# jonassibbesen/rpvg

Hardware: AMD Instinct MI355X
Metric: read-pairs quantified/sec (higher is better)
Workload: dtype f64

## Files before the change

### rpvg_amd/csrc/bounded_search.hip

```cpp

#include "common.hpp"

#include <algorithm>
#include <cstdlib>
#include <map>
#include <memory>
#include <mutex>
#include <numeric>

using namespace rpvg_hip_detail;

namespace {
std::mutex g_search_gate_mutex;
const rpvg_hip_ctx * g_search_gate_owner = nullptr;
}

static bool searchLaunchesEarly() {
    static const bool early = RPVG_EXPERIMENT_ENV("RPVG_HIP_SEARCH_LAUNCH_EARLY") != nullptr;
    return early;
}

constexpr uint64_t kSearchGateRows = 1ull << 17;

static void searchGateEnter(rpvg_hip_ctx * ctx, hipStream_t stream, const uint64_t matrix_rows) {
    static const bool open_gate = RPVG_EXPERIMENT_ENV("RPVG_HIP_NO_SEARCH_GATE") != nullptr;
    ctx->search_gate_held = !open_gate && matrix_rows >= kSearchGateRows;
    if (!ctx->search_gate_held) return;
    hipEvent_t previous = nullptr;
    {
        std::lock_guard<std::mutex> lock(g_search_gate_mutex);
        if (g_search_gate_owner && g_search_gate_owner != ctx && g_search_gate_owner->device == ctx->device) {
            previous = g_search_gate_owner->search_done;
            (void) hipStreamWaitEvent(stream, previous, 0);
        }
    }
    if (previous && !searchLaunchesEarly()) (void) waitEvent(previous);
}

static void searchGateLeave(rpvg_hip_ctx * ctx, hipStream_t stream) {
    if (!ctx->search_gate_held) return;
    ctx->search_gate_held = false;
    std::lock_guard<std::mutex> lock(g_search_gate_mutex);
    (void) hipEventRecord(ctx->search_done, stream);
    g_search_gate_owner = ctx;
}

void searchGateForget(const rpvg_hip_ctx * ctx) {
    std::lock_guard<std::mutex> lock(g_search_gate_mutex);
    if (g_search_gate_owner == ctx) g_search_gate_owner = nullptr;
}

struct rpvg_hip_pair_posteriors {
    std::vector<uint64_t> pair_off;
    void * block = nullptr;
    bool block_pinned = false;
    const uint32_t * first = nullptr, * second = nullptr;
    const double * posterior = nullptr;
    ~rpvg_hip_pair_posteriors() {
        if (block && block_pinned) pinnedFree(block);
        else std::free(block);
    }
};

namespace {

constexpr uint32_t kLdsRows = 2048;
constexpr uint32_t kSmallRows = 512;
constexpr uint32_t kSmallRowLdsCols = 128;
constexpr uint32_t kRowLdsCols = 512;

__device__ __forceinline__ double waveSum(double v) { return waveSumF64(v); }

__device__ __forceinline__ double addLog(const double log_x, const double log_y) {
    return log_x > log_y ? log_x + log1p(exp(log_y - log_x)) : log_y + log1p(exp(log_x - log_y));
}


template <int kBlock, typename ValueFn>
__device__ __forceinline__ double blockLogSumExp(const uint32_t n, ValueFn value, double * scratch) {
    const double lowest = -1.7976931348623157e308;
    const int lane = threadIdx.x & 63, wave = threadIdx.x >> 6;
    double mx = lowest;
    for (uint32_t k = threadIdx.x; k < n; k += kBlock) mx = fmax(mx, value(k));
#pragma unroll
    for (int d = 32; d >= 1; d >>= 1) mx = fmax(mx, __shfl_xor(mx, d, 64));
    __syncthreads();
    if (lane == 0) scratch[wave] = mx;
    __syncthreads();
#pragma unroll
    for (int w2 = 0; w2 < kBlock / 64; ++w2) mx = fmax(mx, scratch[w2]);
    double sum = 0.0;
    for (uint32_t k = threadIdx.x; k < n; k += kBlock) {
        const double v = value(k);
        if (v > lowest) sum += exp(v - mx);
    }
    sum = waveSum(sum);
    __syncthreads();
    if (lane == 0) scratch[wave] = sum;
    __syncthreads();
    double total = 0.0;
#pragma unroll
    for (int w2 = 0; w2 < kBlock / 64; ++w2) total += scratch[w2];
    return (n == 0 || !(mx > lowest)) ? lowest : mx + log(total);
}

struct SearchArgs {
    const uint32_t * order;
    uint32_t count;
    const uint64_t * mat_val_off;
    const uint64_t * mat_row_off;
    const uint32_t * mat_fast;
    const uint32_t * mat_mid;
    const uint64_t * mat_rows;
    const uint32_t * mat_cols;
    const double * values;
    const double * rowmax;
    const double * row_count;
    const double * row_noise;
    const uint64_t * col_off;
// ... 1057 lines not shown
        pack.add(d_big_pair_part_off, big_pair_part_off.data(), M);
    }
    const uint32_t evals_word = (M + 1) & ~1u, tail_words = evals_word + 4;
    w.evals_word = evals_word;
    w.tail_words = tail_words;
    auto & d_tail = w.d_tail;
    pack.addZero(d_tail, tail_words);
    if (w.extra_u64_count) pack.add(w.d_extra_u64, w.extra_u64, w.extra_u64_count);
    if (w.extra_zero_bytes) pack.addZero(w.d_extra_zero, w.extra_zero_bytes);
    int span = ctx->spanBegin(FAM_H2D);
    ok(pack.commit(st));
    if (!column_counts) d_col_count.borrow(const_cast<uint32_t *>(groups->d_column_counts), col_off[M]);
    ctx->spanEnd(span);
    ctx->stats.h2d_bytes += static_cast<double>(M * 20 + col_off[M] * 4);
    ok(d_lf.alloc(col_off[M]));
    ok(d_marg.alloc(col_off[M]));
    ok(d_opt_raw.alloc(col_off[M]));
    ok(d_opt.alloc(col_off[M]));
    ok(d_col_order.alloc(col_off[M]));
    ok(d_out_first.alloc(pair_cap_off[M]));
    ok(d_out_second.alloc(pair_cap_off[M]));
    ok(d_out_value.alloc(pair_cap_off[M]));
    if (e != hipSuccess) {
        setError("rpvg_hip_bounded_pair_posteriors: %s", hipGetErrorString(e));
        return (e == hipErrorOutOfMemory) ? RPVG_HIP_ERR_ALLOC : RPVG_HIP_ERR_RUNTIME;
    }

    SearchArgs args;
    args.order = d_order.ptr;
    args.count = M;
    args.mat_val_off = groups->mat_val_off.ptr;
    args.mat_row_off = groups->mat_row_off.ptr;
    args.mat_fast = groups->mat_fast.ptr;
    args.mat_mid = groups->mat_mid.ptr;
    args.mat_rows = groups->mat_rows.ptr;
    args.mat_cols = groups->mat_cols.ptr;
    args.values = groups->values.ptr;
    args.rowmax = groups->rowmax.ptr;
    args.row_count = groups->row_count.ptr;
    args.row_noise = groups->row_noise.ptr;
    args.col_off = d_col_off.ptr;
    args.col_count = d_col_count.ptr;
    args.pair_cap_off = d_pair_cap_off.ptr;
    args.min_log_likelihood_diff = std::log(min_rel_likelihood);
    args.log_freq = d_lf.ptr;
    args.marginal = d_marg.ptr;
    args.optimistic_raw = d_opt_raw.ptr;
    args.optimistic = d_opt.ptr;
    args.col_order = d_col_order.ptr;
    args.out_first = d_out_first.ptr;
    args.out_second = d_out_second.ptr;
    args.out_value = d_out_value.ptr;
    args.out_count = d_tail.ptr;

    args.log_evals = reinterpret_cast<unsigned long long *>(d_tail.ptr + evals_word);
    auto & d_part_marg = w.d_part_marg; auto & d_part_opt = w.d_part_opt; auto & d_part_pair = w.d_part_pair; auto & d_seq = w.d_seq;
    if (num_big > 0) {
        ok(d_part_marg.alloc(col_part_total));
        ok(d_part_opt.alloc(col_part_total));
        ok(d_part_pair.alloc(pair_part_total));
        ok(d_seq.alloc(pair_cap_off[M]));
    }
    if (e != hipSuccess) {
        setError("rpvg_hip_bounded_pair_posteriors: %s", hipGetErrorString(e));
        return (e == hipErrorOutOfMemory) ? RPVG_HIP_ERR_ALLOC : RPVG_HIP_ERR_RUNTIME;
    }

    static const int search_streams = []() {
        const char * env = RPVG_EXPERIMENT_ENV("RPVG_HIP_SEARCH_STREAMS");
        return env ? std::max(1, std::min(3, std::atoi(env))) : 3;
    }();
    hipStream_t s_medium = search_streams == 1 ? st : ctx->aux[0];
    hipStream_t s_small = search_streams == 1 ? st : (search_streams == 2 ? ctx->aux[0] : ctx->aux[1]);
    const bool side_kernels = M > num_big;
    const bool runs_behind_search = static_cast<bool>(groups->held_back_runs) && pair_tiles && num_big == M;
    if (!runs_behind_search) {
        ok(groups->waitCollapse(st));
        if (groups->collapse_done && !searchLaunchesEarly()) {
            HostScope wait_scope("search: wait for the collapse of the matrices");
            ok(waitEvent(groups->collapse_done));
        }
    }
    span = ctx->spanBegin(FAM_LOGLIK);
    searchGateEnter(ctx, st, std::accumulate(groups->h_num_rows.begin(), groups->h_num_rows.end(), uint64_t(0)));
    if (side_kernels) ok(ctx->forkAux());
    if (num_big > 0) {
        TableWork tw;
        tw.item_matrix = d_item_matrix.ptr;
        tw.item_col = d_item_col.ptr;
        tw.item_chunk = d_item_chunk.ptr;
        tw.count = static_cast<uint32_t>(item_matrix.size());
        tw.mat_val_off = groups->mat_val_off.ptr;
        tw.mat_row_off = groups->mat_row_off.ptr;
        tw.mat_fast = groups->mat_fast.ptr;
        tw.mat_mid = groups->mat_mid.ptr;
        tw.mat_rows = groups->mat_rows.ptr;
        tw.mat_cols = groups->mat_cols.ptr;
        tw.values = groups->values.ptr;
        tw.rowmax = groups->rowmax.ptr;
        tw.row_count = groups->row_count.ptr;
        tw.row_noise = groups->row_noise.ptr;
        tw.big_col_part_off = d_big_col_part_off.ptr;
        tw.big_pair_part_off = d_big_pair_part_off.ptr;
        tw.part_marginal = d_part_marg.ptr;
        tw.part_optimistic = d_part_opt.ptr;
        tw.part_pair = d_part_pair.ptr;
        tw.log_evals = args.log_evals;
        if (pair_tiles) {
            PairTileWork pw;
            pw.item_matrix = d_item_matrix.ptr;
            pw.item_chunk = d_item_chunk.ptr;
            pw.item_tiles = d_item_col.ptr;
            pw.chunk_rows = chunk_rows;
            pw.count = tw.count;
            pw.mat_val_off = groups->mat_val_off.ptr;
            pw.mat_row_off = groups->mat_row_off.ptr;
            pw.mat_fast = groups->mat_fast.ptr;
            pw.mat_mid = groups->mat_mid.ptr;
            pw.mat_rows = groups->mat_rows.ptr;
            pw.mat_cols = groups->mat_cols.ptr;
            pw.values = groups->values.ptr;
            pw.row_count = groups->row_count.ptr;
            pw.row_noise = groups->row_noise.ptr;
            pw.col_part_off = d_big_col_part_off.ptr;
            pw.pair_part_off = d_big_pair_part_off.ptr;
            pw.part_marginal = d_part_marg.ptr;
            pw.part_pair = d_part_pair.ptr;
            pw.log_evals = args.log_evals;
#ifdef RPVG_HIP_EXPERIMENTS
            pw.debug_skip = RPVG_EXPERIMENT_ENV("RPVG_HIP_PAIR_DEBUG") ? static_cast<uint32_t>(std::atoi(RPVG_EXPERIMENT_ENV("RPVG_HIP_PAIR_DEBUG"))) : 0u;
#endif
            static const size_t tile_lds_bytes = []() {
                const char * env = RPVG_EXPERIMENT_ENV("RPVG_HIP_PAIR_LDS_KB");
                return std::max<size_t>(kTileLdsDoubles * sizeof(double), env ? static_cast<size_t>(std::atoi(env)) * 1024 : 0);
            }();
            if (tile_lds_bytes > 64 * 1024) {
                RPVG_HIP_CHECK(hipFuncSetAttribute(reinterpret_cast<const void *>(&pairTile2Kernel), hipFuncAttributeMaxDynamicSharedMemorySize, static_cast<int>(tile_lds_bytes)));
            }
            const int tile_span = ctx->spanBegin(FAM_TILE, st);
            pairTile2Kernel<<<dim3(pw.count), dim3(kTileBlock), tile_lds_bytes, st>>>(pw);
            ctx->spanEnd(tile_span);
#ifdef RPVG_HIP_EXPERIMENTS
            for (int k = RPVG_EXPERIMENT_ENV("RPVG_HIP_PAIR_REPEAT") ? std::atoi(RPVG_EXPERIMENT_ENV("RPVG_HIP_PAIR_REPEAT")) : 0; k > 0; --k) {
                pairTile2Kernel<<<dim3(pw.count), dim3(kTileBlock), tile_lds_bytes, st>>>(pw);
            }
#endif
        } else {
            pairTableKernel<<<dim3(((tw.count + 7) / 8) * 8), dim3(256), 0, st>>>(tw);
        }
        if (runs_behind_search && e == hipSuccess) {
            if (groups->collapse_done) {
                HostScope wait_scope("search: wait for the runs of the matrices' collapse");
                ok(searchLaunchesEarly() ? hipStreamWaitEvent(st, groups->collapse_done, 0) : waitEvent(groups->collapse_done));
            }
            rpvg_hip_groups::SearchSums sums;
            sums.part_pair = d_part_pair.ptr;
            sums.part_marginal = d_part_marg.ptr;
            sums.pair_part_off = d_big_pair_part_off.ptr;
            sums.col_part_off = d_big_col_part_off.ptr;
            sums.chunk_rows = chunk_rows;
            ok(groups->held_back_runs(st, &sums));
            groups->held_back_runs = nullptr;
        }

        ResolveArgs ra;
        ra.big_matrix = d_order.ptr;
        ra.count = num_big;
        ra.mat_rows = groups->mat_rows.ptr;
        ra.mat_cols = groups->mat_cols.ptr;
        ra.chunk_rows = chunk_rows;
        ra.col_off = d_col_off.ptr;
        ra.col_count = d_col_count.ptr;
        ra.pair_cap_off = d_pair_cap_off.ptr;
        ra.big_col_part_off = d_big_col_part_off.ptr;
        ra.big_pair_part_off = d_big_pair_part_off.ptr;
        ra.part_marginal = d_part_marg.ptr;
        ra.part_optimistic = d_part_opt.ptr;
        ra.part_pair = d_part_pair.ptr;
        ra.min_log_likelihood_diff = args.min_log_likelihood_diff;
        ra.log_freq = d_lf.ptr;
        ra.marginal = d_marg.ptr;
        ra.col_order = d_col_order.ptr;
        ra.seq_value = d_seq.ptr;
        ra.out_first = d_out_first.ptr;
        ra.out_second = d_out_second.ptr;
        ra.out_value = d_out_value.ptr;
        ra.out_count = d_tail.ptr;
        resolveTableKernel<<<dim3(num_big), dim3(256), 0, st>>>(ra);
    }
    args.row_lds_cols = kRowLdsCols;
    auto search_lds_bytes = [](uint32_t stage_rows, uint32_t row_cols) { return static_cast<size_t>((kTileFirst + 1) * stage_rows + kTileFirst * row_cols) * sizeof(double); };
    {
        static std::once_flag once;
        std::call_once(once, [&]() {
            (void) hipFuncSetAttribute(reinterpret_cast<const void *>(&boundedSearchKernel<1024, 64>), hipFuncAttributeMaxDynamicSharedMemorySize,
                                       static_cast<int>(search_lds_bytes(kLdsRows, kRowLdsCols)));
        });
    }
    if (num_medium > 0) {
        args.order = d_order.ptr + num_big;
        args.count = num_medium;
        args.stage_rows = kLdsRows;
        boundedSearchKernel<1024, 64><<<dim3(num_medium), dim3(1024), search_lds_bytes(kLdsRows, kRowLdsCols), s_medium>>>(args);
    }
    if (M > num_big + num_medium) {
        args.order = d_order.ptr + num_big + num_medium;
        args.count = M - num_big - num_medium;
        args.stage_rows = kSmallRows;
        args.row_lds_cols = kSmallRowLdsCols;
        boundedSearchKernel<256, 16><<<dim3(args.count), dim3(256), search_lds_bytes(kSmallRows, kSmallRowLdsCols), s_small>>>(args);
    }
    if (side_kernels) ok(ctx->joinAux());
    ctx->spanEnd(span);
    ctx->stats.loglik_launches += (num_big > 0 ? 2 : 0) + (num_medium > 0) + (M > num_big + num_medium);
    ok(hipGetLastError());
    if (e != hipSuccess) {
        setError("rpvg_hip_bounded_pair_posteriors: %s", hipGetErrorString(e));
        (void) hipStreamSynchronize(st);
        return RPVG_HIP_ERR_RUNTIME;
    }
    return RPVG_HIP_OK;
}

void leavePairSearch(rpvg_hip_ctx * ctx) { searchGateLeave(ctx, ctx->stream); }

void accountPairSearch(rpvg_hip_ctx * ctx, const rpvg_hip_groups * groups, const PairSearchWork & w, const unsigned long long log_evals,
                       const uint64_t kept_pairs) {
    ctx->stats.loglik_evals += static_cast<double>(log_evals);
    for (uint32_t i = 0; i < w.M; ++i) {
        const double G = groups->h_num_cols[w.order[i]];
        ctx->stats.search_pairs_possible += G * (G + 1) / 2;
        if (i < w.num_big) ctx->stats.search_pairs_table += G * (G + 1) / 2;
    }
    ctx->stats.search_pairs_kept += static_cast<double>(kept_pairs);
}

}

extern "C" int rpvg_hip_bounded_pair_posteriors(rpvg_hip_ctx * ctx, const rpvg_hip_groups * groups,
                                                const uint32_t * column_counts, double min_rel_likelihood,
                                                rpvg_hip_pair_posteriors ** result_out) {
    RPVG_REQUIRE(ctx && groups && result_out, "rpvg_hip_bounded_pair_posteriors: NULL argument");
    *result_out = nullptr;
    RPVG_REQUIRE(min_rel_likelihood > 0, "rpvg_hip_bounded_pair_posteriors: min_rel_likelihood must be positive");
    const uint32_t M = groups->num_matrices;
    rpvg_hip_pair_posteriors * res = new (std::nothrow) rpvg_hip_pair_posteriors();
    if (!res) {
        setError("rpvg_hip_bounded_pair_posteriors: out of host memory");
        return RPVG_HIP_ERR_ALLOC;
    }
    res->pair_off.assign(M + 1, 0);
    if (M == 0) {
        *result_out = res;
        return RPVG_HIP_OK;
    }
    if (!column_counts && !groups->d_column_counts) {
        delete res;
        setError("rpvg_hip_bounded_pair_posteriors: column_counts is NULL");
        return RPVG_HIP_ERR_INVALID;
    }

    std::lock_guard<std::mutex> lock(ctx->mutex);
    PairSearchWork w;
    {
        const int rc = queuePairSearch(ctx, groups, column_counts, min_rel_likelihood, w);
        if (rc != RPVG_HIP_OK) {
            delete res;
            return rc;
        }
    }
    hipError_t e = hipSuccess;
    hipStream_t st = ctx->stream;
    auto ok = [&](hipError_t r) { if (e == hipSuccess) e = r; return e == hipSuccess; };
    std::unique_ptr<HostScope> scope;
    const std::vector<uint64_t> & pair_cap_off = w.pair_cap_off;
    const uint32_t evals_word = w.evals_word, tail_words = w.tail_words;
    auto & d_tail = w.d_tail; auto & d_pair_cap_off = w.d_pair_cap_off; auto & d_out_first = w.d_out_first;
    auto & d_out_second = w.d_out_second; auto & d_out_value = w.d_out_value;
    DeviceBuffer<uint64_t> d_pair_off;

    const char * with_counts_env = std::getenv("RPVG_HIP_PAIRS_WITH_COUNTS");
    const size_t kPairsWithTheCounts = with_counts_env ? static_cast<size_t>(std::atof(with_counts_env)) : (size_t(1) << 20);
    const size_t tail_bytes = tail_words * sizeof(uint32_t), tail_room = (tail_bytes + 255) & ~size_t(255);
    const size_t block_capacity = static_cast<size_t>(pair_cap_off[M]) * 16;
    const size_t first_copy = tail_room + std::min(block_capacity, kPairsWithTheCounts);
    DeviceBuffer<unsigned char> d_result;
    ok(d_pair_off.alloc(M + 1));
    ok(d_result.alloc(tail_room + block_capacity));
    void * host_result = nullptr;
    if (e == hipSuccess && pinnedAlloc(&host_result, first_copy) != hipSuccess) e = hipErrorOutOfMemory;
    if (e == hipSuccess) {
        const bool check_build = !groups->build_checked && groups->build_error_flag.ptr;
        pairOffsetsKernel<<<dim3(1), dim3(1024), 0, st>>>(M, d_tail.ptr, d_pair_off.ptr, check_build ? groups->build_error_flag.ptr : nullptr,
                                                         d_tail.ptr + evals_word + 2, reinterpret_cast<uint32_t *>(d_result.ptr), tail_words);
        compactPairsBlockKernel<<<dim3(M), dim3(64), 0, st>>>(M, d_pair_cap_off.ptr, d_pair_off.ptr, d_out_first.ptr, d_out_second.ptr,
                                                             d_out_value.ptr, d_result.ptr + tail_room);
        ok(hipGetLastError());
        ok(hipMemcpyAsync(host_result, d_result.ptr, first_copy, hipMemcpyDeviceToHost, st));
    }
    searchGateLeave(ctx, st);
    scope.reset(new HostScope("bounded search: wait for the kernels"));
    ok(waitStream(st));
    if (e == hipSuccess) {
        const uint32_t * counts = static_cast<const uint32_t *>(host_result);
        unsigned long long log_evals = 0;
        std::memcpy(&log_evals, counts + evals_word, sizeof(log_evals));
        const uint32_t build_bad = counts[evals_word + 2];
// ... 58 lines not shown
```

### rpvg_amd/csrc/common.hpp

```cpp
#ifndef RPVG_HIP_COMMON_HPP
#define RPVG_HIP_COMMON_HPP

#include <hip/hip_runtime.h>

#include <algorithm>
#include <chrono>
#include <cstdarg>
#include <cstdint>
#include <cstdio>
#include <cstdlib>
#include <cstring>
#include <memory>
#include <mutex>
#include <new>
#include <string>
#include <functional>
#include <vector>

#include "../../include/rpvg_hip.h"

namespace rpvg_hip_detail {

void setError(const char * fmt, ...);

// ... 415 lines not shown
    }
}

constexpr int kCollapseKeyFractionBits = 22;
constexpr int kCollapseProjectionBits = kCollapseKeyFractionBits + 2;
constexpr int kCollapseLargestBits = 20;
constexpr int kCollapseLargestFractionBits = 27;
constexpr int kCollapseMatrixShift = kCollapseProjectionBits + kCollapseLargestBits;
constexpr uint32_t kCollapseMaxMatrices = 1u << 20;

__host__ __device__ inline double collapseWeight(const uint32_t column) {
    return static_cast<double>(((column * 0x9E3779B1u) >> 8) & 0xFFFFu) * (1.0 / 32768.0);
}

__host__ __device__ inline uint64_t collapseSortKey(const uint32_t matrix, const double key, const double largest) {
    const double k = key < 0.0 ? 0.0 : (key > 3.999999 ? 3.999999 : key);
    const double l = largest < 0.0 ? 0.0 : (largest > 0.999999 ? 0.999999 : largest);
    return (static_cast<uint64_t>(matrix) << kCollapseMatrixShift) |
           (static_cast<uint64_t>(k * static_cast<double>(1ull << kCollapseKeyFractionBits)) << kCollapseLargestBits) |
           (static_cast<uint64_t>(l * static_cast<double>(1ull << kCollapseLargestFractionBits)) & ((1ull << kCollapseLargestBits) - 1));
}

__device__ __forceinline__ double mulRounded(const double a, const double b) {
#pragma clang fp contract(off)
    return a * b;
}
__device__ __forceinline__ double addRounded(const double a, const double b) {
#pragma clang fp contract(off)
    return a + b;
}

template <int BLOCK>
__device__ __forceinline__ uint32_t blockExclusiveSum(const uint32_t v, uint32_t & total, uint32_t * scratch) {
    const int lane = threadIdx.x & 63, wave = threadIdx.x >> 6;
    uint32_t incl = v;
#pragma unroll
    for (int d = 1; d < 64; d <<= 1) {
        const uint32_t up = __shfl_up(incl, d, 64);
        if (lane >= d) incl += up;
    }
    __syncthreads();
    if (lane == 63) scratch[wave] = incl;
    __syncthreads();
    uint32_t before = 0, all = 0;
#pragma unroll
    for (int w = 0; w < BLOCK / 64; ++w) {
        if (w < wave) before += scratch[w];
        all += scratch[w];
    }
    total = all;
    return before + incl - v;
}

enum KernelFamily { FAM_EM_SPARSE = 0, FAM_EM_DENSE, FAM_LOGLIK, FAM_BUILD, FAM_H2D, FAM_COLLAPSE, FAM_EM_KERNEL, FAM_GIBBS, FAM_TILE, FAM_COUNT };

struct TimedSpan {
    hipEvent_t start, stop;
    int family;
    int sub;
};

struct TimedInterval {
    double start_ms, stop_ms;
    int family;
    uint64_t clock;
};

}

namespace rpvg_hip_detail {
struct SubsetEmHints {
    double subsets_per_matrix = 0, list_per_path = 0, rows_per_row = 0, entries_per_entry = 0;
    bool retry = false;
    unsigned long long retry_subsets = 0, retry_list_length = 0, retry_rows = 0, retry_entries = 0;
};
}

struct rpvg_hip_ctx {
    static constexpr int kAuxStreams = 6;
    rpvg_hip_detail::SubsetEmHints subset_hints;
    bool search_gate_held = false;
    int device = 0;
    hipStream_t stream = nullptr;
    hipStream_t aux[kAuxStreams] = {};
    int aux_count = kAuxStreams;
    hipStream_t grid_stream[2] = {nullptr, nullptr};
    hipEvent_t grid_ready = nullptr;
    hipStream_t collapse_stream = nullptr;
    hipStream_t copy_stream = nullptr;
    hipEvent_t copied = nullptr;
    hipEvent_t fork_event = nullptr;
    hipEvent_t search_done = nullptr;
    hipEvent_t join_event[kAuxStreams] = {};
    hipError_t forkAux();
    hipError_t joinAux();
    hipError_t joinAuxOnHost();
    hipDeviceProp_t props;
    std::mutex mutex;
    void * comm = nullptr;
    int comm_world = 1, comm_rank = 0;
    int allReduceSumF64(double * device_buf, uint64_t n);
    std::vector<rpvg_hip_detail::TimedSpan> spans;
    std::vector<hipStream_t> span_streams;
    int span_level = 2;
    int open_spans = 0;
    void accountSpan(const rpvg_hip_detail::TimedSpan & span, const void * clock_base, uint64_t clock_id);
    void foldFinishedSpans();
    std::vector<rpvg_hip_detail::TimedInterval> intervals;
    rpvg_hip_kernel_stats stats;

    int spanBegin(int family, hipStream_t on = nullptr, int sub = -1);
    void spanEnd(int idx);
    int foldSpans();
};

namespace rpvg_hip_detail {
struct PathSourcesPending {
    DeviceBuffer<uint64_t> d_path_source_off;
    DeviceBuffer<uint32_t> d_source_id, d_sizes;
    DeviceBuffer<uint16_t> d_source_id16;
    DeviceBuffer<unsigned long long> d_arena;
    unsigned long long arena_words = 0, num_sources = 0, num_sources_narrow = 0;
    void * h_sizes = nullptr;
    uint32_t K = 0;
    bool copied = false, queued = false;
    ~PathSourcesPending() { if (h_sizes) pinnedFree(h_sizes); }
};
}

struct rpvg_hip_batch {
    uint32_t num_clusters = 0;
    uint64_t num_rows = 0, num_entries = 0, num_paths = 0;
    std::vector<uint64_t> h_cluster_row_off, h_cluster_path_off, h_cluster_ent_off;
    rpvg_hip_detail::DeviceBuffer<uint64_t> cluster_row_off;
    rpvg_hip_detail::DeviceBuffer<uint64_t> cluster_path_off;
    rpvg_hip_detail::DeviceBuffer<double> row_count;
    rpvg_hip_detail::DeviceBuffer<double> row_noise;
    rpvg_hip_detail::DeviceBuffer<uint64_t> row_ent_off;
    rpvg_hip_detail::DeviceBuffer<uint32_t> ent_path;
    rpvg_hip_detail::DeviceBuffer<double> ent_prob;
    std::vector<double> h_cluster_total;
    bool has_source_columns = false;
    rpvg_hip_detail::DeviceBuffer<uint32_t> path_group_id;
    rpvg_hip_detail::DeviceBuffer<uint64_t> cluster_src_off;
    rpvg_hip_detail::DeviceBuffer<uint32_t> src_col_count;
    rpvg_hip_detail::DeviceBuffer<uint32_t> src_col_end;
    rpvg_hip_detail::DeviceBuffer<uint32_t> src_col_path;
    std::vector<uint64_t> h_cluster_src_off;
    std::vector<uint32_t> h_src_num_cols, h_src_col_paths, h_src_max_col_paths;
    struct UploadInProgress {
        rpvg_hip_detail::DeviceBuffer<uint32_t> d_row_count_u32, d_row_grp_off32, d_grp_idx_off32;
        rpvg_hip_detail::DeviceBuffer<uint64_t> d_row_grp_off, d_grp_idx_off;
        rpvg_hip_detail::DeviceBuffer<double> d_grp_prob;
        rpvg_hip_detail::DeviceBuffer<uint8_t> d_row_grp_count8, d_grp_idx_count8;
        rpvg_hip_detail::DeviceBuffer<uint16_t> d_path_idx16, d_row_noise16;
        rpvg_hip_detail::DeviceBuffer<double> d_row_noise_table;
        rpvg_hip_detail::DeviceBuffer<uint8_t> d_row_count8;
        rpvg_hip_detail::DeviceBuffer<uint32_t> d_escape_row, d_escape_count;
        uint64_t num_groups = 0;
        rpvg_hip_detail::PathSourcesPending path_sources;
        rpvg_hip_detail::DeviceBuffer<unsigned long long> d_first_bad_row;
        rpvg_hip_detail::DeviceBuffer<double> d_cluster_total;
        rpvg_hip_detail::DeviceBuffer<uint64_t> d_cluster_ent_off;
        rpvg_hip_detail::DeviceBuffer<unsigned char> scan_scratch_rows, scan_scratch_groups;
        void * h_results = nullptr;
        hipEvent_t finished = nullptr;
// ... 126 lines not shown
    uint32_t num_fused = 0;
    hipEvent_t filled = nullptr, collapsed = nullptr, collapse_sorted = nullptr;
    ~EmSolveWork() {
        if (filled) (void) hipEventDestroy(filled);
        if (collapsed) (void) hipEventDestroy(collapsed);
        if (collapse_sorted) (void) hipEventDestroy(collapse_sorted);
    }
};
size_t emQueuesBytes();
uint32_t emFillSegmentRows();

struct EmGridControl {
    uint32_t done;
    uint32_t iterations;
    uint32_t conv_its;
    uint32_t viol;
    uint32_t error;
    uint32_t arrived;
};

struct EmGridProblem {
    uint32_t problem, columns;
    uint32_t rows, entries;
    uint32_t merged, pad;
    uint64_t row_base, ent_base, col_begin;
    double total_mass, zero_mass;
};

struct EmGridStorage {
    const uint32_t * prow_off;
    const double * prow_count;
    const double * merged_count;
    const double * prow_noise;
    const uint32_t * pent_col;
    const double * pent_val;
    double * abundances;
    double * noise_count;
    uint32_t * iterations;
    const EmFusedDense * fused = nullptr;
    uint32_t num_fused = 0;
};

uint64_t emGridMinWork();
bool emGridDenseRoute(uint32_t columns, uint32_t rows, uint32_t entries);
int runEmGridProblems(rpvg_hip_ctx * ctx, hipStream_t st, const EmGridProblem * problems, uint32_t count, const EmGridStorage & storage,
                      uint32_t max_em_its, double max_rel_em_conv);

struct DenseEmRun {
    const double * matrix = nullptr;
    uint64_t num_rows = 0;
    uint32_t num_cols = 0;
    uint64_t ld = 0;
    const double * counts = nullptr;
    double total_count = 0, zero_mass = 0;
    uint32_t max_em_its = 0;
    double max_rel_em_conv = 0;
    bool sharded = false;
    DeviceBuffer<double> d_a;
    EmGridControl control = {};
};
int emDenseIterate(rpvg_hip_ctx * ctx, const char * who, DenseEmRun & run);

int queueEmSolve(rpvg_hip_ctx * ctx, const rpvg_hip_batch * batch, const EmProblemList & list, uint32_t max_em_its,
                 double max_rel_em_conv, const EmOutputs & out, EmSolveWork & work, bool fill_only, double collapse_precision = 0.0);
void accountEmSolve(rpvg_hip_ctx * ctx, uint32_t P, const uint64_t * col_off, const uint32_t * kept_rows, const uint32_t * kept_entries,
                    const uint32_t * iterations);

struct PairSearchWork {
    uint32_t M = 0, num_big = 0, evals_word = 0, tail_words = 0;
    std::vector<uint32_t> order;
    std::vector<uint64_t> col_off, pair_cap_off;
    DeviceBuffer<uint32_t> d_order, d_col_count, d_col_order, d_out_first, d_out_second, d_item_matrix, d_item_col, d_item_chunk;
    DeviceBuffer<uint32_t> d_tail;
    DeviceBuffer<uint64_t> d_col_off, d_pair_cap_off, d_big_col_part_off, d_big_pair_part_off;
    DeviceBuffer<double> d_lf, d_marg, d_opt_raw, d_opt, d_out_value, d_part_marg, d_part_opt, d_part_pair, d_seq;
    UploadPack pack;
    const uint64_t * extra_u64 = nullptr;
    size_t extra_u64_count = 0, extra_zero_bytes = 0;
    DeviceBuffer<uint64_t> d_extra_u64;
    DeviceBuffer<unsigned char> d_extra_zero;
};
int queuePairSearch(rpvg_hip_ctx * ctx, const rpvg_hip_groups * groups, const uint32_t * column_counts, double min_rel_likelihood,
                    PairSearchWork & w);
void leavePairSearch(rpvg_hip_ctx * ctx);
void accountPairSearch(rpvg_hip_ctx * ctx, const rpvg_hip_groups * groups, const PairSearchWork & w, unsigned long long log_evals, uint64_t kept_pairs);

struct CsrCollapseInput {
    uint32_t num_problems_bound = 0;
    const uint32_t * num_problems_dev = nullptr;
    uint64_t rows_capacity = 0;
    const uint64_t * row_base = nullptr;
    const uint64_t * ent_base = nullptr;
    const uint32_t * kept_rows = nullptr;
    const uint64_t * col_off = nullptr;
    const uint32_t * prow_off = nullptr;
    const double * prow_count = nullptr;
    const double * prow_noise = nullptr;
    const uint32_t * pent_col = nullptr;
    const double * pent_val = nullptr;
    uint32_t num_items_bound = 0;
    const uint32_t * num_items_dev = nullptr;
    const uint64_t * seg_first = nullptr;
    const uint32_t * item_problem = nullptr;
    uint32_t segment_rows = 0;
    uint64_t max_rows_bound = 0;
};
struct CsrCollapseWork {
    DeviceBuffer<double> merged_count;
    DeviceBuffer<uint32_t> problem_merged;
    DeviceBuffer<uint32_t> info;
    std::shared_ptr<void> temporaries;
};
hipError_t queueCsrCollapse(rpvg_hip_ctx * ctx, const CsrCollapseInput & in, double precision, CsrCollapseWork & work, hipStream_t stream,
                            hipEvent_t sorted = nullptr);

hipError_t queueClusterTotals(hipStream_t stream, uint32_t num_clusters, const uint64_t * d_cluster_row_off, const uint32_t * d_row_count_u32, double * d_totals);
hipError_t queuePathSourceCopies(rpvg_hip_ctx * ctx, rpvg_hip_batch * b, const rpvg_cluster_batch * hb, PathSourcesPending & pending);
hipError_t queuePathSourceKernels(rpvg_hip_ctx * ctx, rpvg_hip_batch * b, PathSourcesPending & pending, hipStream_t stream);
hipError_t reservePathSources(rpvg_hip_batch * b, uint32_t num_clusters, uint64_t num_paths, uint64_t num_sources, PathSourcesPending & pending);
int finishPathSources(rpvg_hip_batch * b, PathSourcesPending & pending);

hipError_t queueRowCollapse(rpvg_hip_ctx * ctx, rpvg_hip_groups * groups, uint64_t total_rows, double precision, hipStream_t stream, bool hold_back_runs = false);
}

#endif
```

### rpvg_amd/csrc/context.hip

```cpp

#include "common.hpp"

#include <hipcub/hipcub.hpp>

#include <sys/prctl.h>
#include <time.h>

#include <algorithm>
#include <thread>

#include <map>

namespace rpvg_hip_detail {

static thread_local char g_last_error[1024] = "";

void setError(const char * fmt, ...) {
    va_list ap;
    va_start(ap, fmt);
    vsnprintf(g_last_error, sizeof(g_last_error), fmt, ap);
    va_end(ap);
}

namespace {
// ... 443 lines not shown
template <typename GrpOff>
__global__ void expandGroupsKernel(const uint64_t num_groups, const uint64_t num_entries, const GrpOff * __restrict__ grp_idx_off,
                                   const double * __restrict__ grp_prob, double * __restrict__ ent_prob) {
    const uint64_t g = blockIdx.x * static_cast<uint64_t>(blockDim.x) + threadIdx.x;
    if (g >= num_groups) return;
    const double p = grp_prob[g];
    for (uint64_t e = grp_idx_off[g]; e < min(static_cast<uint64_t>(grp_idx_off[g + 1]), num_entries); ++e) ent_prob[e] = p;
}

template <typename RowOff, typename GrpOff>
__global__ void rowMetaKernel(const uint64_t num_rows, const uint64_t num_groups, const RowOff * __restrict__ row_grp_off,
                              const GrpOff * __restrict__ grp_idx_off, const uint32_t * __restrict__ row_count_u32,
                              uint64_t * __restrict__ row_ent_off, double * __restrict__ row_count) {
    const uint64_t r = blockIdx.x * static_cast<uint64_t>(blockDim.x) + threadIdx.x;
    if (r > num_rows) return;
    row_ent_off[r] = grp_idx_off[min(static_cast<uint64_t>(row_grp_off[r]), num_groups)];
    if (r < num_rows) row_count[r] = static_cast<double>(row_count_u32[r]);
}

template <typename RowOff, typename GrpOff>
__global__ void validateRowsKernel(const uint64_t num_rows, const uint64_t num_groups, const uint64_t num_entries, const uint32_t num_clusters,
                                   const uint64_t * __restrict__ cluster_row_off, const uint64_t * __restrict__ cluster_path_off,
                                   const RowOff * __restrict__ row_grp_off, const GrpOff * __restrict__ grp_idx_off,
                                   const double * __restrict__ row_noise, const uint32_t * __restrict__ path_idx,
                                   unsigned long long * __restrict__ first_bad_row) {
    const uint64_t r = blockIdx.x * static_cast<uint64_t>(blockDim.x) + threadIdx.x;
    if (r >= num_rows) return;
    bool good = true;
    const uint64_t g0 = row_grp_off[r], g1 = row_grp_off[r + 1];
    good = g0 <= g1 && g1 <= num_groups;
    const double nz = row_noise[r];
    good = good && nz > 0 && nz <= 1;
    if (good) {
        uint32_t lo = 0, hi = num_clusters;
        while (hi - lo > 1) {
            const uint32_t mid = lo + (hi - lo) / 2;
            if (cluster_row_off[mid] <= r) lo = mid;
            else hi = mid;
        }
        const uint64_t n_paths = cluster_path_off[lo + 1] - cluster_path_off[lo];
        uint64_t e = grp_idx_off[g0];
        good = e <= num_entries;
        for (uint64_t g = g0; good && g < g1; ++g) {
            const uint64_t e1 = grp_idx_off[g + 1];
            good = e <= e1 && e1 <= num_entries;
            for (; good && e < e1; ++e) good = path_idx[e] < n_paths;
        }
    }
    if (!good) atomicMin(first_bad_row, static_cast<unsigned long long>(r));
}

extern "C" {

int rpvg_hip_device_count(int * count) {
    RPVG_REQUIRE(count != nullptr, "rpvg_hip_device_count: count is NULL");
    int n = 0;
    hipError_t e = hipGetDeviceCount(&n);
    if (e != hipSuccess) {
        setError("hipGetDeviceCount failed: %s", hipGetErrorString(e));
        *count = 0;
        return RPVG_HIP_ERR_NO_DEVICE;
    }
    *count = n;
    return RPVG_HIP_OK;
}

namespace {
hipError_t createMainStream(hipStream_t * stream, const bool highest_priority) {
    const char * env = RPVG_EXPERIMENT_ENV("RPVG_HIP_MAIN_PRIORITY");
    if (!highest_priority && (!env || std::atoi(env) == 0)) return hipStreamCreateWithFlags(stream, hipStreamNonBlocking);
    int least = 0, greatest = 0;
    if (hipDeviceGetStreamPriorityRange(&least, &greatest) != hipSuccess || least == greatest) {
        (void) hipGetLastError();
        return hipStreamCreateWithFlags(stream, hipStreamNonBlocking);
    }
    return hipStreamCreateWithPriority(stream, hipStreamNonBlocking, greatest);
}

bool ownQueueForMainStream(const bool uploader, const int side_streams) {
    static const bool pooled = std::getenv("RPVG_HIP_POOLED_MAIN_QUEUE") != nullptr && std::atoi(std::getenv("RPVG_HIP_POOLED_MAIN_QUEUE")) != 0;
    return !uploader && side_streams < rpvg_hip_ctx::kAuxStreams && !pooled;
}

hipError_t createOwnQueueStream(hipStream_t * stream, const int num_cus) {
    uint32_t every_cu[32];
    for (uint32_t & word : every_cu) word = 0xffffffffu;
    const uint32_t words = static_cast<uint32_t>(std::min(32, std::max(1, (num_cus + 31) / 32)));
    hipError_t e = hipExtStreamCreateWithCUMask(stream, words, every_cu);
    if (e != hipSuccess) {
        (void) hipGetLastError();
        e = hipStreamCreateWithFlags(stream, hipStreamNonBlocking);
    }
    return e;
}

int createContext(int device, bool uploader, int side_streams, rpvg_hip_ctx ** ctx_out);
}

int rpvg_hip_create(int device, rpvg_hip_ctx ** ctx_out) { return createContext(device, false, rpvg_hip_ctx::kAuxStreams, ctx_out); }

int rpvg_hip_create_uploader(int device, rpvg_hip_ctx ** ctx_out) { return createContext(device, true, 1, ctx_out); }

int rpvg_hip_create_with_streams(int device, int side_streams, rpvg_hip_ctx ** ctx_out) {
    RPVG_REQUIRE(side_streams >= 1 && side_streams <= rpvg_hip_ctx::kAuxStreams, "rpvg_hip_create_with_streams: 1 to %d side streams", rpvg_hip_ctx::kAuxStreams);
    return createContext(device, false, side_streams, ctx_out);
}

namespace {
int createContext(int device, const bool uploader, const int side_streams, rpvg_hip_ctx ** ctx_out) {
    RPVG_REQUIRE(ctx_out != nullptr, "rpvg_hip_create: ctx_out is NULL");
    *ctx_out = nullptr;
    int n = 0;
    hipError_t e = hipGetDeviceCount(&n);
    if (e != hipSuccess || n <= 0) {
        setError("rpvg_hip_create: no HIP device available (%s); this engine has no CPU fallback",
                 e != hipSuccess ? hipGetErrorString(e) : "device count is 0");
        return RPVG_HIP_ERR_NO_DEVICE;
    }
    RPVG_REQUIRE(device >= 0 && device < n, "rpvg_hip_create: device %d out of range [0, %d)", device, n);
    rpvg_hip_ctx * ctx = new (std::nothrow) rpvg_hip_ctx();
    if (!ctx) {
        setError("rpvg_hip_create: out of host memory");
        return RPVG_HIP_ERR_ALLOC;
    }
    ctx->device = device;
    memset(&ctx->stats, 0, sizeof(ctx->stats));
    {
        const char * env = std::getenv("RPVG_HIP_SPANS");
        ctx->span_level = env ? std::max(0, std::min(2, std::atoi(env))) : ((uploader || side_streams < rpvg_hip_ctx::kAuxStreams) ? 1 : 2);
    }
    if ((e = hipSetDevice(device)) != hipSuccess || (e = hipGetDeviceProperties(&ctx->props, device)) != hipSuccess ||
        (e = ownQueueForMainStream(uploader, side_streams) ? createOwnQueueStream(&ctx->stream, ctx->props.multiProcessorCount) : createMainStream(&ctx->stream, uploader)) != hipSuccess) {
        setError("rpvg_hip_create: %s", hipGetErrorString(e));
        delete ctx;
        return RPVG_HIP_ERR_RUNTIME;
    }
    ctx->aux_count = side_streams;
    for (int i = 0; i < rpvg_hip_ctx::kAuxStreams && e == hipSuccess; ++i) {
        if (i < side_streams) {
            e = hipStreamCreateWithFlags(&ctx->aux[i], hipStreamNonBlocking);
            if (e == hipSuccess) e = hipEventCreateWithFlags(&ctx->join_event[i], hipEventDisableTiming);
        } else {
            ctx->aux[i] = ctx->aux[i % side_streams];
        }
    }
    if (e == hipSuccess) e = createMainStream(&ctx->collapse_stream, RPVG_EXPERIMENT_ENV("RPVG_HIP_COLLAPSE_PRIORITY") == nullptr || std::atoi(RPVG_EXPERIMENT_ENV("RPVG_HIP_COLLAPSE_PRIORITY")) != 0);
    if (e == hipSuccess) e = hipEventCreateWithFlags(&ctx->fork_event, hipEventDisableTiming);
    if (e == hipSuccess) e = hipEventCreateWithFlags(&ctx->search_done, hipEventDisableTiming);
    if (e == hipSuccess) e = hipStreamCreateWithFlags(&ctx->copy_stream, hipStreamNonBlocking);
    if (e == hipSuccess) e = hipEventCreateWithFlags(&ctx->copied, hipEventDisableTiming);
    if (e == hipSuccess) {
        registerCopyStream(ctx->stream, ctx->copy_stream, ctx->copied);
        for (int i = 0; i < ctx->aux_count; ++i) registerCopyStream(ctx->aux[i], ctx->copy_stream, ctx->copied);
    }
    if (e != hipSuccess) {
        setError("rpvg_hip_create: %s", hipGetErrorString(e));
        delete ctx;
        return RPVG_HIP_ERR_RUNTIME;
    }
    if (strncmp(ctx->props.gcnArchName, "gfx950", 6) != 0) {
        setError("rpvg_hip_create: device %d is %s; this library is built for gfx950 only", device, ctx->props.gcnArchName);
        (void) hipStreamDestroy(ctx->stream);
        delete ctx;
        return RPVG_HIP_ERR_NO_DEVICE;
    }
    {
        std::lock_guard<std::mutex> lock(g_pool_mutex);
        g_device_contexts[device]++;
    }
    *ctx_out = ctx;
    return RPVG_HIP_OK;
}
}

void rpvg_hip_destroy(rpvg_hip_ctx * ctx) {
    if (!ctx) return;
    const bool trace = std::getenv("RPVG_AMD_TRACE_EXIT") != nullptr;
#define RPVG_EXIT_STEP(what) do { if (trace) std::fprintf(stderr, "[exit]   rpvg_hip_destroy: %s\n", what); } while (0)
    RPVG_EXIT_STEP("begin");
    (void) hipSetDevice(ctx->device);
    (void) ctx->foldSpans();
    RPVG_EXIT_STEP("spans folded");
    (void) rpvg_hip_comm_destroy(ctx);
    if (ctx->stream) forgetCopyStream(ctx->stream);
    for (int i = 0; i < ctx->aux_count; ++i) {
        if (ctx->aux[i]) forgetCopyStream(ctx->aux[i]);
    }
    if (ctx->copy_stream) {
        (void) hipStreamSynchronize(ctx->copy_stream);
        (void) hipStreamDestroy(ctx->copy_stream);
    }
    RPVG_EXIT_STEP("copy stream destroyed");
    if (ctx->copied) (void) hipEventDestroy(ctx->copied);
    if (ctx->stream) (void) hipStreamSynchronize(ctx->stream);
    for (int i = 0; i < ctx->aux_count; ++i) {
        if (ctx->aux[i]) (void) hipStreamSynchronize(ctx->aux[i]);
    }
    if (ctx->collapse_stream) (void) hipStreamSynchronize(ctx->collapse_stream);
    RPVG_EXIT_STEP("streams drained");
    for (int i = 0; i < ctx->aux_count; ++i) {
        if (ctx->aux[i]) (void) hipStreamDestroy(ctx->aux[i]);
        RPVG_EXIT_STEP("a side stream destroyed");
        if (ctx->join_event[i]) (void) hipEventDestroy(ctx->join_event[i]);
    }
    if (ctx->collapse_stream) (void) hipStreamDestroy(ctx->collapse_stream);
    RPVG_EXIT_STEP("side and collapse streams destroyed");
    if (ctx->stream) (void) hipStreamDestroy(ctx->stream);
    RPVG_EXIT_STEP("main stream destroyed");
    if (ctx->fork_event) (void) hipEventDestroy(ctx->fork_event);
    for (hipStream_t grid_stream : ctx->grid_stream) {
        if (grid_stream) {
            (void) hipStreamSynchronize(grid_stream);
            (void) hipStreamDestroy(grid_stream);
        }
    }
// ... 897 lines not shown
```

### rpvg_amd/csrc/subset_em.hip

```cpp

#include "common.hpp"

#include <cmath>
#include <memory>

using namespace rpvg_hip_detail;

namespace {

constexpr uint32_t kMaxSelected = 1024;

struct MergedList {
    const uint32_t * a;
    const uint32_t * b;
    uint32_t na, nb, i, j;
    __device__ __forceinline__ MergedList(const uint32_t * a_in, uint32_t na_in, const uint32_t * b_in, uint32_t nb_in)
        : a(a_in), b(b_in), na(na_in), nb(nb_in), i(0), j(0) {}
    __device__ __forceinline__ bool done() const { return i >= na && j >= nb; }
    __device__ __forceinline__ uint32_t next() {
        if (j >= nb || (i < na && a[i] <= b[j])) return a[i++];
        return b[j++];
    }
};

// ... 790 lines not shown
    ok(d_slot_columns.alloc(slots));
    ok(d_slot_weight.alloc(slots));
    ok(d_totals.alloc(sizeof(MatrixTotals) * M));
    ok(d_bases.alloc(sizeof(MatrixTotals) * M));
    DeviceBuffer<uint32_t> d_big_matrices;
    ok(d_big_matrices.alloc(M));
    DeviceBuffer<uint32_t> d_sub_cluster, d_path, d_col_path, d_iters, d_kept_rows, d_kept_entries;
    DeviceBuffer<double> d_sub_weight, d_abund, d_noise, d_total;
    DeviceBuffer<uint64_t> d_path_off, d_col_off, d_row_base, d_ent_base, d_subset_off, d_seg_first;
    DeviceBuffer<uint32_t> d_item_problem;
    ok(d_sub_cluster.alloc(cap_subsets));
    ok(d_sub_weight.alloc(cap_subsets));
    ok(d_path_off.alloc(cap_subsets + 1));
    ok(d_col_off.alloc(cap_subsets + 1));
    ok(d_row_base.alloc(cap_subsets));
    ok(d_ent_base.alloc(cap_subsets));
    ok(d_subset_off.alloc(M + 1));
    ok(d_seg_first.alloc(cap_subsets + 1));
    ok(d_item_problem.alloc(cap_items));
    ok(d_path.alloc(cap_length));
    ok(d_col_path.alloc(cap_columns));
    ok(d_abund.alloc(cap_columns));
    ok(d_noise.alloc(cap_subsets));
    ok(d_total.alloc(cap_subsets));
    ok(d_iters.alloc(cap_subsets));
    ok(d_kept_rows.alloc(cap_subsets));
    ok(d_kept_entries.alloc(cap_subsets));
    const size_t packed_capacity = packedLayout(M, cap_subsets, cap_length, cap_columns).bytes;
    ok(d_packed.alloc(packed_capacity));
    const bool merge_here = batch->path_group_id.ptr != nullptr && max_paths < (1u << kMergePathBits) - 2;
    DeviceBuffer<unsigned long long> d_merge_key;
    DeviceBuffer<uint32_t> d_merge_pos;
    DeviceBuffer<double> d_merge_a0, d_merge_a1;
    if (merge_here) {
        ok(d_merge_key.alloc(2 * cap_length + 2));
        ok(d_merge_pos.alloc(2 * cap_length + 2));
        ok(d_merge_a0.alloc(cap_length));
        ok(d_merge_a1.alloc(cap_length));
    }
    void * pinned_header = nullptr;
    if (e == hipSuccess && pinnedAlloc(&pinned_header, sizeof(SubsetHeader)) != hipSuccess) e = hipErrorOutOfMemory;
    hipEvent_t header_here = nullptr;
    if (e == hipSuccess) ok(hipEventCreateWithFlags(&header_here, hipEventDisableTiming));
    if (e != hipSuccess) {
        setError("rpvg_hip_nested_subset_em: %s", hipGetErrorString(e));
        (void) hipStreamSynchronize(st);
        leavePairSearch(ctx);
        if (pinned_header) pinnedFree(pinned_header);
        if (header_here) (void) hipEventDestroy(header_here);
        return (e == hipErrorOutOfMemory) ? RPVG_HIP_ERR_ALLOC : RPVG_HIP_ERR_RUNTIME;
    }
    MatrixTotals * totals = reinterpret_cast<MatrixTotals *>(d_totals.ptr);
    MatrixTotals * bases = reinterpret_cast<MatrixTotals *>(d_bases.ptr);

    std::unique_ptr<HostScope> part_scope(new HostScope("subset em: select + offsets + expand queued"));
    int span = ctx->spanBegin(FAM_BUILD);
    SelectArgs sa;
    sa.num_matrices = M;
    sa.pair_count = search.d_tail.ptr;
    sa.pair_cap_off = search.d_pair_cap_off.ptr;
    sa.pair_first = search.d_out_first.ptr;
    sa.pair_second = search.d_out_second.ptr;
    sa.pair_value = search.d_out_value.ptr;
    sa.group_off = groups->d_group_off;
    sa.group_path_off = groups->d_group_path_off;
    sa.group_path = groups->d_group_path;
    sa.cluster = groups->d_cluster;
    sa.mat_rows = groups->mat_rows.ptr;
    sa.cluster_row_off = batch->cluster_row_off.ptr;
    sa.row_ent_off = batch->row_ent_off.ptr;
    sa.slot_off = d_slot_off;
    sa.min_hap_prob = min_hap_prob;
    sa.segment_rows = emFillSegmentRows();
    sa.slot_first = d_slot_first.ptr;
    sa.slot_second = d_slot_second.ptr;
    sa.slot_weight = d_slot_weight.ptr;
    sa.slot_length = d_slot_length.ptr;
    sa.slot_columns = d_slot_columns.ptr;
    sa.totals = totals;
    sa.header = header;
    sa.big_matrices = d_big_matrices.ptr;
    subsetSelectSmallKernel<<<dim3(M), dim3(64), 0, st>>>(sa);
    subsetSelectWideKernel<<<dim3(std::min<uint32_t>(M, 128)), dim3(256), 0, st>>>(sa);
    const bool check_build = !groups->build_checked && groups->build_error_flag.ptr;
    OffsetsArgs oa;
    oa.pair_count = search.d_tail.ptr;
    oa.log_evals = reinterpret_cast<const unsigned long long *>(search.d_tail.ptr + search.evals_word);
    oa.build_error = check_build ? groups->build_error_flag.ptr : nullptr;
    oa.num_matrices = M;
    oa.totals = totals;
    oa.bases = bases;
    oa.header = header;
    oa.cap_subsets = cap_subsets;
    oa.cap_length = cap_length;
    oa.cap_columns = cap_columns;
    oa.cap_rows = cap_rows;
    oa.cap_entries = cap_entries;
    oa.cap_items = cap_items;
    oa.seg_first = d_seg_first.ptr;
    oa.path_off = d_path_off.ptr;
    oa.col_off = d_col_off.ptr;
    subsetOffsetsKernel<<<dim3(1), dim3(1024), 0, st>>>(oa);
    SubsetHeader * h_header = static_cast<SubsetHeader *>(pinned_header);
    ok(hipMemcpyAsync(h_header, header, sizeof(SubsetHeader), hipMemcpyDeviceToHost, st));
    ok(hipEventRecord(header_here, st));
    ExpandArgs ea;
    ea.num_matrices = M;
    ea.header = header;
    ea.totals = totals;
    ea.bases = bases;
    ea.slot_off = d_slot_off;
    ea.slot_first = d_slot_first.ptr;
    ea.slot_second = d_slot_second.ptr;
    ea.slot_weight = d_slot_weight.ptr;
    ea.slot_length = d_slot_length.ptr;
    ea.slot_columns = d_slot_columns.ptr;
    ea.group_off = groups->d_group_off;
    ea.group_path_off = groups->d_group_path_off;
    ea.group_path = groups->d_group_path;
    ea.cluster = groups->d_cluster;
    ea.cluster_row_off = batch->cluster_row_off.ptr;
    ea.row_ent_off = batch->row_ent_off.ptr;
    ea.sub_cluster = d_sub_cluster.ptr;
    ea.sub_weight = d_sub_weight.ptr;
    ea.path_off = d_path_off.ptr;
    ea.path = d_path.ptr;
    ea.col_off = d_col_off.ptr;
    ea.col_path = d_col_path.ptr;
    ea.row_base = d_row_base.ptr;
    ea.ent_base = d_ent_base.ptr;
    ea.seg_first = d_seg_first.ptr;
    ea.item_problem = d_item_problem.ptr;
    ea.segment_rows = emFillSegmentRows();
    ea.subset_off = d_subset_off.ptr;
    subsetExpandKernel<<<dim3(M), dim3(256), 0, st>>>(ea);
    ok(hipGetLastError());
    ctx->spanEnd(span);
    ctx->stats.build_launches += 4;
    leavePairSearch(ctx);

    part_scope.reset();
    EmProblemList list;
    list.P_bound = static_cast<uint32_t>(std::min<unsigned long long>(cap_subsets, 0xfffffffeull));
    list.d_num_problems = &header->num_problems;
    list.d_cluster = d_sub_cluster.ptr;
    list.d_col_off = d_col_off.ptr;
    list.d_col_path = d_col_path.ptr;
    list.d_row_base = d_row_base.ptr;
    list.d_ent_base = d_ent_base.ptr;
    list.rows_capacity = cap_rows;
    list.entries_capacity = cap_entries;
    list.d_seg_first = d_seg_first.ptr;
    list.d_item_problem = d_item_problem.ptr;
    list.items_bound = static_cast<uint32_t>(std::min<unsigned long long>(cap_items, 0xfffffffeull));
    list.d_num_items = &header->num_items;
    list.max_cols = max_paths + 1;
    list.max_cluster_paths = max_paths;
    list.max_cluster_work = max_cluster_work;
    list.wide_capacity = 0;
    EmOutputs out{d_abund.ptr, d_noise.ptr, d_iters.ptr, d_kept_rows.ptr, d_kept_entries.ptr, d_total.ptr};
    EmSolveWork work;
    work.zeroed_queues = search.d_extra_zero.ptr + header_room;
    if (e == hipSuccess) {
        rc = queueEmSolve(ctx, batch, list, max_em_its, max_rel_em_conv, out, work, false, collapse_precision);
        if (rc != RPVG_HIP_OK) {
            (void) hipStreamSynchronize(st);
// ... 173 lines not shown
```

Measured before the change: 2.428 billion.

## Narrow the cross-context search gate to cover only the pair tile kernel

```diff
diff --git a/rpvg_amd/csrc/bounded_search.hip b/rpvg_amd/csrc/bounded_search.hip
--- a/rpvg_amd/csrc/bounded_search.hip
+++ b/rpvg_amd/csrc/bounded_search.hip
@@ -7,6 +7,7 @@
 #include <memory>
 #include <mutex>
 #include <numeric>
+#include <string>
 
 using namespace rpvg_hip_detail;
 
@@ -20,21 +21,55 @@
     return early;
 }
 
+static SearchGatePoint searchGateExtent() {
+    static const SearchGatePoint extent = []() {
+        const char * env = RPVG_EXPERIMENT_ENV("RPVG_HIP_SEARCH_GATE_EXTENT");
+        if (!env) return kGateTile;
+        const std::string name(env);
+        return name == "subsets" ? kGateSubsets : name == "select" ? kGateSelect : name == "resolve" ? kGateResolve : kGateTile;
+    }();
+    return extent;
+}
+
 constexpr uint64_t kSearchGateRows = 1ull << 17;
 
-static void searchGateEnter(rpvg_hip_ctx * ctx, hipStream_t stream, const uint64_t matrix_rows) {
+static const rpvg_hip_ctx * searchGatePredecessor(const rpvg_hip_ctx * ctx) {
+    const rpvg_hip_ctx * owner = g_search_gate_owner;
+    return owner && owner != ctx && owner->device == ctx->device ? owner : nullptr;
+}
+
+static void searchGateEnter(rpvg_hip_ctx * ctx, hipStream_t stream, const uint64_t matrix_rows, std::unique_lock<std::mutex> * hand_over = nullptr) {
     static const bool open_gate = RPVG_EXPERIMENT_ENV("RPVG_HIP_NO_SEARCH_GATE") != nullptr;
     ctx->search_gate_held = !open_gate && matrix_rows >= kSearchGateRows;
     if (!ctx->search_gate_held) return;
+    const bool host_wait = !searchLaunchesEarly() && !(hand_over && ctx->main_stream_own_queue);
     hipEvent_t previous = nullptr;
     {
-        std::lock_guard<std::mutex> lock(g_search_gate_mutex);
-        if (g_search_gate_owner && g_search_gate_owner != ctx && g_search_gate_owner->device == ctx->device) {
-            previous = g_search_gate_owner->search_done;
-            (void) hipStreamWaitEvent(stream, previous, 0);
-        }
-    }
-    if (previous && !searchLaunchesEarly()) (void) waitEvent(previous);
+        std::unique_lock<std::mutex> lock(g_search_gate_mutex);
+        if (const rpvg_hip_ctx * owner = searchGatePredecessor(ctx)) {
+            previous = owner->search_done;
+            if (!hand_over) (void) hipStreamWaitEvent(stream, previous, 0);
+        }
+        if (hand_over && !(previous && host_wait)) {
+            if (previous) (void) hipStreamWaitEvent(stream, previous, 0);
+            *hand_over = std::move(lock);
+            return;
+        }
+    }
+    if (previous && host_wait) (void) waitEvent(previous);
+    if (hand_over) {
+        std::unique_lock<std::mutex> lock(g_search_gate_mutex);
+        if (const rpvg_hip_ctx * owner = searchGatePredecessor(ctx)) (void) hipStreamWaitEvent(stream, owner->search_done, 0);
+        *hand_over = std::move(lock);
+    }
+}
+
+static void searchGateHandOver(rpvg_hip_ctx * ctx, hipStream_t stream, std::unique_lock<std::mutex> & hand_over) {
+    if (!hand_over.owns_lock()) return;
+    (void) hipEventRecord(ctx->search_done, stream);
+    g_search_gate_owner = ctx;
+    ctx->search_gate_held = false;
+    hand_over.unlock();
 }
 
 static void searchGateLeave(rpvg_hip_ctx * ctx, hipStream_t stream) {
@@ -1258,7 +1293,10 @@
         }
     }
     span = ctx->spanBegin(FAM_LOGLIK);
-    searchGateEnter(ctx, st, std::accumulate(groups->h_num_rows.begin(), groups->h_num_rows.end(), uint64_t(0)));
+    const uint64_t gate_rows = std::accumulate(groups->h_num_rows.begin(), groups->h_num_rows.end(), uint64_t(0));
+    const bool gate_is_tile_kernel = pair_tiles && num_big == M && searchGateExtent() == kGateTile;
+    std::unique_lock<std::mutex> gate_hand_over;
+    if (!gate_is_tile_kernel) searchGateEnter(ctx, st, gate_rows);
     if (side_kernels) ok(ctx->forkAux());
     if (num_big > 0) {
         TableWork tw;
@@ -1313,6 +1351,7 @@
             if (tile_lds_bytes > 64 * 1024) {
                 RPVG_HIP_CHECK(hipFuncSetAttribute(reinterpret_cast<const void *>(&pairTile2Kernel), hipFuncAttributeMaxDynamicSharedMemorySize, static_cast<int>(tile_lds_bytes)));
             }
+            if (gate_is_tile_kernel) searchGateEnter(ctx, st, gate_rows, &gate_hand_over);
             const int tile_span = ctx->spanBegin(FAM_TILE, st);
             pairTile2Kernel<<<dim3(pw.count), dim3(kTileBlock), tile_lds_bytes, st>>>(pw);
             ctx->spanEnd(tile_span);
@@ -1321,6 +1360,7 @@
                 pairTile2Kernel<<<dim3(pw.count), dim3(kTileBlock), tile_lds_bytes, st>>>(pw);
             }
 #endif
+            searchGateHandOver(ctx, st, gate_hand_over);
         } else {
             pairTableKernel<<<dim3(((tw.count + 7) / 8) * 8), dim3(256), 0, st>>>(tw);
         }
@@ -1363,6 +1403,7 @@
         ra.out_value = d_out_value.ptr;
         ra.out_count = d_tail.ptr;
         resolveTableKernel<<<dim3(num_big), dim3(256), 0, st>>>(ra);
+        if (pair_tiles && num_big == M) leavePairSearch(ctx, kGateResolve);
     }
     args.row_lds_cols = kRowLdsCols;
     auto search_lds_bytes = [](uint32_t stage_rows, uint32_t row_cols) { return static_cast<size_t>((kTileFirst + 1) * stage_rows + kTileFirst * row_cols) * sizeof(double); };
@@ -1398,7 +1439,9 @@
     return RPVG_HIP_OK;
 }
 
-void leavePairSearch(rpvg_hip_ctx * ctx) { searchGateLeave(ctx, ctx->stream); }
+void leavePairSearch(rpvg_hip_ctx * ctx, const SearchGatePoint point) {
+    if (point == kGateSubsets || searchGateExtent() == point) searchGateLeave(ctx, ctx->stream);
+}
 
 void accountPairSearch(rpvg_hip_ctx * ctx, const rpvg_hip_groups * groups, const PairSearchWork & w, const unsigned long long log_evals,
                        const uint64_t kept_pairs) {
diff --git a/rpvg_amd/csrc/common.hpp b/rpvg_amd/csrc/common.hpp
--- a/rpvg_amd/csrc/common.hpp
+++ b/rpvg_amd/csrc/common.hpp
@@ -521,6 +521,7 @@
     bool search_gate_held = false;
     int device = 0;
     hipStream_t stream = nullptr;
+    bool main_stream_own_queue = false;
     hipStream_t aux[kAuxStreams] = {};
     int aux_count = kAuxStreams;
     hipStream_t grid_stream[2] = {nullptr, nullptr};
@@ -813,7 +814,8 @@
 };
 int queuePairSearch(rpvg_hip_ctx * ctx, const rpvg_hip_groups * groups, const uint32_t * column_counts, double min_rel_likelihood,
                     PairSearchWork & w);
-void leavePairSearch(rpvg_hip_ctx * ctx);
+enum SearchGatePoint { kGateTile = 0, kGateResolve = 1, kGateSelect = 2, kGateSubsets = 3 };
+void leavePairSearch(rpvg_hip_ctx * ctx, SearchGatePoint point = kGateSubsets);
 void accountPairSearch(rpvg_hip_ctx * ctx, const rpvg_hip_groups * groups, const PairSearchWork & w, unsigned long long log_evals, uint64_t kept_pairs);
 
 struct CsrCollapseInput {
diff --git a/rpvg_amd/csrc/context.hip b/rpvg_amd/csrc/context.hip
--- a/rpvg_amd/csrc/context.hip
+++ b/rpvg_amd/csrc/context.hip
@@ -549,11 +549,12 @@
     return !uploader && side_streams < rpvg_hip_ctx::kAuxStreams && !pooled;
 }
 
-hipError_t createOwnQueueStream(hipStream_t * stream, const int num_cus) {
+hipError_t createOwnQueueStream(hipStream_t * stream, const int num_cus, bool * own_queue) {
     uint32_t every_cu[32];
     for (uint32_t & word : every_cu) word = 0xffffffffu;
     const uint32_t words = static_cast<uint32_t>(std::min(32, std::max(1, (num_cus + 31) / 32)));
     hipError_t e = hipExtStreamCreateWithCUMask(stream, words, every_cu);
+    *own_queue = e == hipSuccess;
     if (e != hipSuccess) {
         (void) hipGetLastError();
         e = hipStreamCreateWithFlags(stream, hipStreamNonBlocking);
@@ -597,7 +598,7 @@
         ctx->span_level = env ? std::max(0, std::min(2, std::atoi(env))) : ((uploader || side_streams < rpvg_hip_ctx::kAuxStreams) ? 1 : 2);
     }
     if ((e = hipSetDevice(device)) != hipSuccess || (e = hipGetDeviceProperties(&ctx->props, device)) != hipSuccess ||
-        (e = ownQueueForMainStream(uploader, side_streams) ? createOwnQueueStream(&ctx->stream, ctx->props.multiProcessorCount) : createMainStream(&ctx->stream, uploader)) != hipSuccess) {
+        (e = ownQueueForMainStream(uploader, side_streams) ? createOwnQueueStream(&ctx->stream, ctx->props.multiProcessorCount, &ctx->main_stream_own_queue) : createMainStream(&ctx->stream, uploader)) != hipSuccess) {
         setError("rpvg_hip_create: %s", hipGetErrorString(e));
         delete ctx;
         return RPVG_HIP_ERR_RUNTIME;
diff --git a/rpvg_amd/csrc/subset_em.hip b/rpvg_amd/csrc/subset_em.hip
--- a/rpvg_amd/csrc/subset_em.hip
+++ b/rpvg_amd/csrc/subset_em.hip
@@ -896,6 +896,7 @@
     sa.big_matrices = d_big_matrices.ptr;
     subsetSelectSmallKernel<<<dim3(M), dim3(64), 0, st>>>(sa);
     subsetSelectWideKernel<<<dim3(std::min<uint32_t>(M, 128)), dim3(256), 0, st>>>(sa);
+    leavePairSearch(ctx, kGateSelect);
     const bool check_build = !groups->build_checked && groups->build_error_flag.ptr;
     OffsetsArgs oa;
     oa.pair_count = search.d_tail.ptr;
```

Result: no change. 2.426 billion (-0.1%).
